# resero-labs/latok

Hardware: AMD Instinct MI355X
Metric: input UTF-8 GB/s tokenized (fused feature+split-mask path) (higher is better)
Workload: dtype u64

## Files before the change

latok_amd/csrc/api.cpp:

```cpp
#include <hip/hip_runtime.h>
#include <errno.h>
#include <fcntl.h>
#include <stdarg.h>
#include <stdio.h>
#include <stdlib.h>
#include <string.h>
#include <sys/mman.h>
#include <sys/stat.h>
#include <unistd.h>

#include <algorithm>
#include <array>
#include <atomic>
#include <chrono>
#include <mutex>
#include <new>
#include <string>
#include <thread>
#include <vector>

#include "../../include/latok_hip.h"
#include "corpus_gen.h"
#include "flow_hazards.h"
#include "kernels.h"
// ... 3266 lines not shown
    HIP_TRY(latok::launch_utf8_bytes(cps, n, (unsigned long long*)g.ws.scalar.p, g.stream));
    unsigned long long t = 0;
    HIP_TRY(hipMemcpyAsync(&t, g.ws.scalar.p, 8, hipMemcpyDeviceToHost, g.stream));
    HIP_TRY(hipStreamSynchronize(g.stream));
    *bytes_out = (int64_t)t;
    return LATOK_OK;
}

int latok_debug_set_scan_epoch(unsigned epoch) {
    LATOK_ENTER();
    g.ws.scan_epoch = epoch & 0x3FFFFu;
    return LATOK_OK;
}

extern "C" int latok_debug_limits(int64_t* out, int n) {
    const int64_t v[19] = {latok::kTile, latok::kWPB, latok::kNarrowWPB, latok::kSegMax, latok::kOneSegTiles, latok::kFastTailTiles,
                           kSmallChars, kSmallStrings, latok::kCompressWaves, latok::kFeatWaves, latok::kFeatRound, latok::kFeatRoundTm,
                           latok::kFeatFormThresh, latok::kFeatWinBytes, latok::kHashWaveBytes, latok::scan_small_max(),
                           latok::utf8_block_bytes(), latok::kCountProbeMax, latok::kCountAccEntries};
    if (!out || n < 0) return fail(LATOK_ERR_INVALID, "NULL output");
    const int k = n < 19 ? n : 19;
    for (int i = 0; i < k; ++i) out[i] = v[i];
    return k;
}

extern "C" int latok_debug_terms_limits(int64_t* out, int n) {
    const int64_t v[2] = {latok::kTermsTile, latok::kTermsRowMax};
    if (!out || n < 0) return fail(LATOK_ERR_INVALID, "NULL output");
    const int k = n < 2 ? n : 2;
    for (int i = 0; i < k; ++i) out[i] = v[i];
    return k;
}

extern "C" int latok_debug_wordpiece_limits(int64_t* out, int n) {
    const int64_t v[4] = {latok::kWpBlock, latok::scan_chunk(), kWpMaxPrefix, kWpMaxChars};
    if (!out || n < 0) return fail(LATOK_ERR_INVALID, "NULL output");
    const int k = n < 4 ? n : 4;
    for (int i = 0; i < k; ++i) out[i] = v[i];
    return k;
}

static int put_plan(const latok::LaunchPlan& L, int64_t n_tiles, int64_t* out, int n) {
    const int64_t v[12] = {L.n_cu_eff, L.seg_tiles, L.n_segs, L.rounds, L.grid, L.one_launch ? 0 : L.grid, L.fast_tail, L.pf, L.wpb, L.nw,
                           L.one_launch, n_tiles};
    const int k = n < 12 ? n : 12;
    for (int i = 0; i < k; ++i) out[i] = v[i];
    return k;
}

extern "C" int latok_debug_plan(int64_t n_tiles, int n_cu, int in_flow, int mode, int64_t* out, int n) {
    if (!out || n < 0 || n_tiles < 1 || n_cu < 1 || mode < latok::kModeBits || mode > latok::kModeValuesRules)
        return fail(LATOK_ERR_INVALID, "n_tiles >= 1, n_cu >= 1, mode 0..%d", latok::kModeValuesRules);
    latok::LaunchPlan L;
    latok::plan_launch(n_tiles, n_cu, in_flow != 0, mode, one_segment_enabled(), &L);
    return put_plan(L, n_tiles, out, n);
}

extern "C" int latok_debug_set_plan_cus(int n_cu) {
    LATOK_ENTER();
    int rc = need_init(g);
    if (rc) return rc;
    if (n_cu != 0 && (n_cu < 8 || n_cu > g.n_cu)) return fail(LATOK_ERR_INVALID, "plan CUs must be 0 or 8..%d", g.n_cu);
    g.plan_cus = n_cu;
    return LATOK_OK;
}

// ... 1010 lines not shown
```

latok_amd/csrc/kernels.h:

```cpp
#ifndef LATOK_KERNELS_H
#define LATOK_KERNELS_H
#include <hip/hip_runtime.h>
#include <stdint.h>

#include "split_code.h"

namespace latok {

constexpr int kTile = 4096;
constexpr int kTblShift = 7;
constexpr int kStage1Len = 8705;
constexpr int kStage1Pad = 8720;
constexpr int kStage2Len = 255 * 128;
constexpr int kTablesLdsBytes = kStage1Pad + kStage2Len;
constexpr int kB6Stage1Len = LK_B6_STAGE1_LEN;
constexpr int kB6Stage1Bytes = (kB6Stage1Len * 2 + 1023) / 1024 * 1024;
constexpr int kB6MaxBlocks = 400;
constexpr int kB6Stage2Bytes = kB6MaxBlocks * 64;
constexpr int kB6TablesBytes = kB6Stage1Bytes + kB6Stage2Bytes;
static_assert(kB6Stage1Bytes % 1024 == 0 && kB6Stage2Bytes % 1024 == 0 && kB6Stage1Bytes <= kTablesLdsBytes, "byte space keeps its stage 1 where the other modes keep both stages");
constexpr int kStageBytes = 64 * 80;
constexpr int kWaveLdsBytes = kStageBytes + 16 + 65 * 8 + 8;

constexpr int kModeBits = 0;
// ... 90 lines not shown
__device__ __forceinline__ int64_t device_total(const int64_t* p, int64_t bound) {
    const int64_t t = *p;
    return t < 0 ? 0 : (t > bound ? bound : t);
}
#endif

struct FeatParams {
    const uint8_t* codes;
    const int64_t* row_off;
    int64_t n_str, total, n_tiles;
    const uint64_t* bits;
    const uint64_t* kept;
    const int64_t* tile_rank;
    const int64_t* tile_cnt;
    const uint16_t* word_pref;
    const int64_t* tile_first;
    const uint64_t* space;
    int8_t* features;
    void* spans4;
    bool out32;
    const int64_t* n_tokens_dev;
    int64_t cap;
    DoneSignal done;
    DeviceTotal dt;
};
hipError_t launch_features_tiles(const FeatParams& P, int n_cu, hipStream_t st);

void plan_segments(int64_t n_tiles, int n_cu, int* seg_tiles, int64_t* n_segs);
constexpr int64_t kOneSegTiles = 24;
constexpr int64_t kFastTailTiles = 256;
constexpr int kNarrowWPB = 16;
constexpr int kCpsPrefetchRows = 2;
constexpr int kCpsPrefetchRowsFlow = 6;
struct LaunchPlan {
    int n_cu_eff;
    int seg_tiles;
    int64_t n_segs;
    int64_t rounds;
    int grid;
    int fast_tail;
    int pf;
    int wpb;
    int nw;
    int one_launch;
};
void plan_launch(int64_t n_tiles, int n_cu, bool in_flow, int mode, bool one_launch_ok, LaunchPlan* L);
hipError_t launch_tile_index(const SplitParams& P, hipStream_t st);
hipError_t launch_split_tiles(const SplitParams& P, int mode, const LaunchPlan& L, hipStream_t st);
hipError_t launch_resolve_fix(const SplitParams& P, int mode, const LaunchPlan& L, hipStream_t st);
hipError_t launch_one_segment(const SplitParams& P, int mode, hipStream_t st);
hipError_t launch_small_batch(const SplitParams& P, bool rules, int kind, bool out32, void* counts, void* items, int8_t* features,
                              int64_t* n_items, unsigned long long* done, unsigned long long seq, hipStream_t st);
hipError_t launch_any_nonzero(const int8_t* a1, const int8_t* a2, int64_t n, int* flags, hipStream_t st);

hipError_t launch_parse_matrix(const uint32_t* cps, int64_t n, const uint8_t* t1, const uint8_t* t2cls,
                               const uint16_t* cw, int8_t* out, hipStream_t st);
constexpr int kSmallMatrixChars = 4096;
hipError_t launch_parse_matrix_small(const uint32_t* cps, int n, const uint8_t* t1, const uint8_t* t2cls, const uint16_t* cw,
                                     int8_t* out, unsigned long long* done, unsigned long long seq, hipStream_t st);
hipError_t launch_combine_rows(const uint8_t* m, int64_t stride_r, int64_t stride_c, int64_t cols, const int8_t* idx,
                               int idx_ndim, int irows, int icols, int8_t* out, hipStream_t st,
                               unsigned long long* done = nullptr, unsigned long long seq = 0);
hipError_t launch_small_block_mask(const SplitParams& P, unsigned long long* done, unsigned long long seq, hipStream_t st);
hipError_t launch_rebase_rows(int64_t* row, int64_t n, int64_t base, hipStream_t st);
int64_t scan_blocks(int64_t n);
hipError_t launch_exclusive_scan(const int64_t* in, int64_t n, int64_t* out, int64_t* total, int64_t* block_tot,
                                 hipStream_t st, int64_t* total_host = nullptr);
int64_t count_blocks(int64_t n_words);
int64_t scan_chunk();
hipError_t launch_word_counts_scan(bool spans, const uint64_t* bits, const uint64_t* space, int64_t n_words, int64_t total,
                                   uint64_t* kept, int64_t* tile_cnt, uint16_t* word_pref, int64_t* tile_rank,
                                   unsigned long long* chain, unsigned* ticket, unsigned epoch, int64_t* total_dev,
                                   int64_t* total_host, int* err, hipStream_t st, DeviceTotal dt = DeviceTotal{nullptr, nullptr});
hipError_t launch_string_counts(bool out32, const uint64_t* mask, const int64_t* tile_rank, const uint16_t* word_pref,
// ... 108 lines not shown
```

latok_amd/csrc/split_kernels.hip:

```cpp
#include <hip/hip_runtime.h>
#include <stdint.h>
#include <stdlib.h>

#include "bitscan.h"
#include "feat_records.h"
#include "kernels.h"
#include "tile_core.h"

namespace latok {

#ifdef LATOK_STAMPS
__device__ unsigned long long g_stamp_sum[16];
__device__ unsigned long long g_stamp_cnt;
#endif

__device__ __forceinline__ Fn64 fn_then(Fn64 f1, Fn64 f2) {
    Fn64 f;
    const bool c1 = f1.a <= kNegInf64, c2 = f2.a <= kNegInf64;
    if (c2) { f.a = kNegInf64; f.b = f2.b; return f; }
    f.a = c1 ? kNegInf64 : f1.a + f2.a;
    const long long c = f1.b + f2.a;
    f.b = c > f2.b ? c : f2.b;
    return f;
}
// ... 203 lines not shown
            for (int j = 0; j < kLazyPer; ++j) {
                const int row = g * kLazyPer + j;
                if (row < kLazyRows)
                    __builtin_amdgcn_global_load_lds((gptr_t)(P.t1 + 1024 * row + 16 * lane), (lptr_t)(L.tables + 1024 * row), 16, 0, 0);
            }
            __builtin_amdgcn_s_waitcnt(0x0F70);
        }
        __hip_atomic_fetch_add(&L.ctl[1], 1, __ATOMIC_RELEASE, __HIP_MEMORY_SCOPE_WORKGROUP);
    }
    while (__hip_atomic_load(&L.ctl[1], __ATOMIC_ACQUIRE, __HIP_MEMORY_SCOPE_WORKGROUP) < 64 * kLazyGrabs) __builtin_amdgcn_s_sleep(2);
}

template <int MODE = kModeBits>
__device__ __forceinline__ TileLds wave_lds(uint8_t* lds, int wave) {
    TileLds L;
    L.t1 = lds;
    L.t2 = lds + kStage1Pad;
    uint8_t* const w = lds + lds_shift(MODE);
    uint8_t* mine = wave < kWPB ? w + kLdsWaves + wave * kWaveLdsBytes : lds + lds_total(MODE) + (wave - kWPB) * kWaveLdsBytes;
    L.stage = mine;
    L.halo = mine + kStageBytes;
    L.bw = reinterpret_cast<lk_u64*>(mine + kStageBytes + 16);
    L.lut = lds;
    L.ltab = lds + kLdsLeadTab;
    L.tables = lds;
    L.ctl = reinterpret_cast<int*>(w + kLdsMisc) + 16;
    L.t1b = lds;
    L.t2b = lds + kB6Stage1Bytes;
    L.ctab = mode_base(MODE) == kModeBytes ? lds + kLdsByteCodes : L.lut + kSliceLutBytes;
    L.small_bits = L.small_space = nullptr;
    return L;
}

template <int MODE, bool FAST_TAIL = false, int WPB = kWPB, int PF = kCpsPrefetchRows>
__device__ __forceinline__ void run_segment(const SplitParams& P, uint8_t* lds, int64_t seg, int tid, int lane,
                                            int wave, bool tables LATOK_STAMP_PARAM) {
    const int S = P.seg_tiles;
    const TileLds L = wave_lds<MODE>(lds, wave);
    int4* sm = reinterpret_cast<int4*>(lds + lds_shift(MODE) + kLdsSumm);
    ScanLdsT<WPB>& scan = *reinterpret_cast<ScanLdsT<WPB>*>(lds + lds_shift(MODE) + kLdsScan);

    const int64_t T0 = seg * S;
    const int64_t T1 = min(T0 + S, P.n_tiles);
    const int n_seg = (int)(T1 - T0);
    int64_t tfv = 0;
    if (wave + WPB * lane < n_seg) tfv = P.tile_first[T0 + wave + WPB * lane];
    tfv = tfv < 0 ? 0 : (tfv > P.n_str ? P.n_str : tfv);
    if (tables) __syncthreads();
    constexpr bool kDefer = mode_writes_bits(MODE) && !mode_is_bytes(MODE);
    lk_u64 obuf[8];
    int slot = 0, k_first = wave;
    const int64_t n_words = (P.total + 63) >> 6;
    auto flush = [&]() {
#pragma unroll
        for (int j = 0; j < 8; ++j) {
            if (j < slot) {
                const int64_t w = (T0 + k_first + j * WPB) * 64 + lane;
                if (w < n_words) P.bits_out[w] = obuf[j];
            }
        }
        slot = 0;
    };
    auto put = [&](lk_u64 w, int k) {
        if (slot == 0) k_first = k;
#pragma unroll
        for (int j = 0; j < 8; ++j) obuf[j] = (j == slot) ? w : obuf[j];
        if (++slot == 8) flush();
    };
    CpsPrefetch pf;
    pf.valid = false;
    for (int k = wave, j = 0; k < n_seg; k += WPB, ++j) {
        const lk_u64 w = process_tile<MODE, kDefer, false, FAST_TAIL, PF>(P, L, T0 + k, lane_read64(tfv, j), 0, -1, true, &sm[k], lane LATOK_STAMP_ARG
                                                                      , MODE == kModeBits && !FAST_TAIL ? &pf : nullptr, k + WPB < n_seg ? T0 + k + WPB : (int64_t)-1
                                                                      );
        if (kDefer) put(w, k);
#ifdef LATOK_STAMPS
        stamp_acc[0] += 1;
#endif
    }
    if (kDefer) flush();
    __syncthreads();
    {
        Fn64 f = fn_identity();
        Hd64 h = hd_identity();
        if (tid < n_seg) {
            const int4 s = sm[tid];
            P.summ[T0 + tid] = s;
            f = fn_of(s);
            h.h = s.z; h.c = s.w & 1;
        }
        Fn64 ef, tfn; Hd64 eh, th;
        block_scan<WPB>(f, h, scan, &ef, &eh, &tfn, &th);
        if (tid == 0) { P.seg_fn[seg] = tfn; P.seg_hd[seg] = th; }
    }
    __syncthreads();
}

template <int MODE, bool FAST_TAIL = false, int PF = kCpsPrefetchRows>
__global__ __launch_bounds__(tile_wpb(MODE) * 64) void k_tiles_main(SplitParams P) {
    constexpr int WPB = tile_wpb(MODE);
    __shared__ __attribute__((aligned(16))) uint8_t lds[lds_total_tiles(MODE)];
    const int tid = threadIdx.x;
    const int lane = tid & 63;
    const int wave = __builtin_amdgcn_readfirstlane(tid >> 6);
    if (blockIdx.x == 0 && tid == 0) *P.fix_count = 0;

    bool tables = MODE != kModeBlockMask;
    if (tables) {
        if (mode_base(MODE) == kModeBytes) load_tables_ascii_bytes(lds, P);
        else load_tables<WPB * 64, MODE>(lds, P);
    }
#ifdef LATOK_STAMPS
    unsigned long long stamp_acc[16];
    for (int i = 0; i < 16; ++i) stamp_acc[i] = 0;
#endif
    for (int64_t seg = blockIdx.x; seg < P.n_segs; seg += gridDim.x) {
        run_segment<MODE, FAST_TAIL, WPB, PF>(P, lds, seg, tid, lane, wave, tables LATOK_STAMP_ARG);
        tables = false;
    }
#ifdef LATOK_STAMPS
    if (lane == 0)
        for (int i = 0; i < 16; ++i) atomicAdd(&g_stamp_sum[i], stamp_acc[i]);
#endif
}

template <int MODE, int NW, bool ONE>
__device__ __forceinline__ void resolve_segments(const SplitParams& P, uint8_t* lds, int tid, int lane, int wave) {
    const int S = P.seg_tiles;
    ScanLdsT<NW>& scan = *reinterpret_cast<ScanLdsT<NW>*>(lds + lds_shift(MODE) + kLdsScan);
    int* misc = reinterpret_cast<int*>(lds + lds_shift(MODE) + kLdsMisc);
    int* fix_t = reinterpret_cast<int*>(lds + lds_shift(MODE) + kLdsTf);
    int2* fix_in = reinterpret_cast<int2*>(lds + lds_shift(MODE) + kLdsSumm);
    bool tables_loaded = ONE;

    for (int64_t seg = ONE ? 0 : (int64_t)blockIdx.x; seg < (ONE ? 1 : P.n_segs); seg += ONE ? 1 : (int64_t)gridDim.x) {
        const int64_t T0 = seg * S;
        const int64_t T1 = min(T0 + S, P.n_tiles);
        const int n_seg = (int)(T1 - T0);
        if (tid == 0) misc[0] = 0;
        const int64_t t = T0 + tid;
        int4 s = make_int4(0, 0, 0, 0);
        if (tid < n_seg) s = P.summ[t];
        Fn64 pf = fn_identity();
        Hd64 sh = hd_identity();
        if (P.n_segs > 1) {
            const int64_t per = (P.n_segs + NW * 64 - 1) / (NW * 64);
            const int64_t lo = min((int64_t)tid * per, P.n_segs), hi = min(lo + per, P.n_segs);
            Fn64 f = fn_identity();
            Hd64 h = hd_identity();
            for (int64_t j = lo; j < hi; ++j) {
// ... 411 lines not shown
    if (s > kSegMax) s = kSegMax;
    *seg_tiles = (int)s;
    *n_segs = (n_tiles + s - 1) / s;
}

void plan_launch(int64_t n_tiles, int n_cu, bool in_flow, int mode, bool one_launch_ok, LaunchPlan* L) {
    const int wpb = tile_wpb(mode);
    int n_cu_eff = n_cu;
    if (in_flow && n_cu >= 64) {
        const int cand[3] = {n_cu * 7 / 8, n_cu * 13 / 16, n_cu * 3 / 4};
        int best = cand[0], best_fill = -1;
        for (int c = 0; c < 3; ++c) {
            int st_ = 0;
            int64_t ns_ = 0;
            plan_segments(n_tiles, cand[c], &st_, &ns_);
            const int fill = (st_ - 1) % wpb + 1;
            if (fill * 2 >= wpb) { best = cand[c]; break; }
            if (fill > best_fill) { best = cand[c]; best_fill = fill; }
        }
        n_cu_eff = best;
    }
    if (n_cu_eff < 8) n_cu_eff = n_cu < 8 ? n_cu : 8;
    L->n_cu_eff = n_cu_eff;
    plan_segments(n_tiles, n_cu_eff, &L->seg_tiles, &L->n_segs);
    L->one_launch = one_launch_ok && n_tiles <= kOneSegTiles && (mode == kModeBits || mode == kModeRules);
    if (L->one_launch) {
        L->seg_tiles = (int)(n_tiles < kOneSegTiles ? kOneSegTiles : n_tiles);
        L->n_segs = 1;
    }
    L->grid = L->one_launch ? 1 : (int)(L->n_segs < n_cu ? (L->n_segs < 1 ? 1 : L->n_segs) : n_cu);
    L->rounds = (L->n_segs + L->grid - 1) / L->grid;
    L->fast_tail = !L->one_launch && n_tiles <= kFastTailTiles && (mode == kModeBits || mode == kModeRules);
    L->pf = mode == kModeBits && in_flow && !L->fast_tail && !L->one_launch ? kCpsPrefetchRowsFlow : kCpsPrefetchRows;
    L->wpb = L->one_launch ? kWPB : wpb;
    const bool narrow_resolve = mode == kModeBits || mode == kModeBytes || mode == kModeLatin1 || mode == kModeUcs2;
    L->nw = L->one_launch || !narrow_resolve ? kWPB : (L->seg_tiles <= 128 ? 2 : (L->seg_tiles <= 256 ? 4 : kWPB));
}

hipError_t launch_split_tiles(const SplitParams& P, int mode, const LaunchPlan& L, hipStream_t st) {
    const dim3 grid(L.grid), block(kWPB * 64);
    if (mode == kModeBits && L.pf == kCpsPrefetchRowsFlow) hipLaunchKernelGGL((k_tiles_main<kModeBits, false, kCpsPrefetchRowsFlow>), grid, block, 0, st, P);
    else if (mode == kModeBits && L.fast_tail) hipLaunchKernelGGL((k_tiles_main<kModeBits, true>), grid, block, 0, st, P);
    else if (mode == kModeRules && L.fast_tail) hipLaunchKernelGGL((k_tiles_main<kModeRules, true>), grid, block, 0, st, P);
    else if (mode == kModeBits) hipLaunchKernelGGL((k_tiles_main<kModeBits>), grid, block, 0, st, P);
    else if (mode == kModeValues) hipLaunchKernelGGL((k_tiles_main<kModeValues>), grid, block, 0, st, P);
    else if (mode == kModeRules) hipLaunchKernelGGL((k_tiles_main<kModeRules>), grid, block, 0, st, P);
    else if (mode == kModeBytes) hipLaunchKernelGGL((k_tiles_main<kModeBytes>), grid, dim3(tile_wpb(kModeBytes) * 64), 0, st, P);
    else if (mode == kModeLatin1) hipLaunchKernelGGL((k_tiles_main<kModeLatin1>), grid, dim3(tile_wpb(kModeLatin1) * 64), 0, st, P);
    else if (mode == kModeUcs2) hipLaunchKernelGGL((k_tiles_main<kModeUcs2>), grid, dim3(tile_wpb(kModeUcs2) * 64), 0, st, P);
    else if (mode == kModeBytesRules) hipLaunchKernelGGL((k_tiles_main<kModeBytesRules>), grid, block, 0, st, P);
    else if (mode == kModeLatin1Rules) hipLaunchKernelGGL((k_tiles_main<kModeLatin1Rules>), grid, block, 0, st, P);
    else if (mode == kModeUcs2Rules) hipLaunchKernelGGL((k_tiles_main<kModeUcs2Rules>), grid, block, 0, st, P);
    else if (mode == kModeValuesRules) hipLaunchKernelGGL((k_tiles_main<kModeValuesRules>), grid, block, 0, st, P);
    else hipLaunchKernelGGL((k_tiles_main<kModeBlockMask>), grid, block, 0, st, P);
    return hipGetLastError();
}

hipError_t launch_one_segment(const SplitParams& P, int mode, hipStream_t st) {
    if (P.n_segs != 1 || P.seg_tiles < P.n_tiles || P.n_tiles > kOneSegTiles || (mode != kModeBits && mode != kModeRules))
        return hipErrorInvalidValue;
    if (mode == kModeBits) hipLaunchKernelGGL((k_one_segment<kModeBits>), dim3(1), dim3(kWPB * 64), 0, st, P);
    else hipLaunchKernelGGL((k_one_segment<kModeRules>), dim3(1), dim3(kWPB * 64), 0, st, P);
    return hipGetLastError();
}

hipError_t launch_resolve_fix(const SplitParams& P, int mode, const LaunchPlan& L, hipStream_t st) {
    if (L.nw * 64 < P.seg_tiles) return hipErrorInvalidValue;
    const dim3 grid(L.grid), block(kWPB * 64);
#define LATOK_RESOLVE_NW(M)                                                                            \
    if (L.nw == 2) hipLaunchKernelGGL((k_resolve_fix<M, 2>), grid, dim3(128), 0, st, P);               \
    else if (L.nw == 4) hipLaunchKernelGGL((k_resolve_fix<M, 4>), grid, dim3(256), 0, st, P);          \
    else hipLaunchKernelGGL((k_resolve_fix<M, kWPB>), grid, block, 0, st, P)
    if (mode == kModeBits) { LATOK_RESOLVE_NW(kModeBits); }
    else if (mode == kModeValues) hipLaunchKernelGGL((k_resolve_fix<kModeValues, kWPB>), grid, block, 0, st, P);
    else if (mode == kModeRules) hipLaunchKernelGGL((k_resolve_fix<kModeRules, kWPB>), grid, block, 0, st, P);
    else if (mode == kModeBytesRules) hipLaunchKernelGGL((k_resolve_fix<kModeBytesRules, kWPB>), grid, block, 0, st, P);
    else if (mode == kModeLatin1Rules) hipLaunchKernelGGL((k_resolve_fix<kModeLatin1Rules, kWPB>), grid, block, 0, st, P);
// ... 23 lines not shown
```

latok_amd/csrc/tile_core.h:

```cpp
#ifndef LATOK_TILE_CORE_H
#define LATOK_TILE_CORE_H
#include <hip/hip_runtime.h>
#include <stdint.h>

#include "kernels.h"
#include "lane_math.h"
#include "utf8_decode.h"
#include "wave_ops.h"

namespace latok {

#ifdef LATOK_STAMPS
#define LATOK_STAMP(k)                                                                           \
    do {                                                                                         \
        __builtin_amdgcn_sched_barrier(0);                                                       \
        unsigned long long t_;                                                                   \
        asm volatile("s_memtime %0\n\ts_waitcnt lgkmcnt(0)" : "=s"(t_)::"memory");            \
        __builtin_amdgcn_sched_barrier(0);                                                       \
        if ((k) > 0) stamp_acc[(k)] += t_ - stamp_prev;                                          \
        stamp_prev = t_;                                                                         \
    } while (0)
#define LATOK_STAMP_ARG , stamp_acc
#define LATOK_STAMP_PARAM , unsigned long long* stamp_acc
#define LATOK_STAMP_NULL , nullptr
// ... 226 lines not shown
    return *reinterpret_cast<const uint2*>(ltab + ((W & 0xFFu) << 3));
}
__device__ __forceinline__ bool lead_index(uint2 q, uint32_t W, uint32_t* off2, uint32_t* R) {
    lk_lead_entry e;
    e.sel = q.x; e.hi0 = q.y;
    uint32_t o;
    const bool bad = lk_lead_index(e, W, &o, R);
    *off2 = min(o, 2u * (uint32_t)(kB6Stage1Len - 1));
    return bad;
}

template <int Q>
__device__ __forceinline__ uint32_t bytes_slot_window(const uint32_t (&w)[5], uint32_t m, uint32_t* r8_out) {
    const uint32_t r8 = (uint32_t)__builtin_ctz(m | 0x80000000u) & 24u;
    *r8_out = r8;
    return __builtin_amdgcn_alignbit(w[Q + 1], w[Q], r8);
}

__device__ __forceinline__ uint32_t bytes_halo_load(const uint8_t* __restrict__ u8, int64_t t0, int64_t total, int lane) {
    uint32_t hb = 0;
    if (lane == 0) {
        if (t0 > 0) hb = *reinterpret_cast<const uint32_t*>(u8 + t0 - 4);
    } else if (lane < 12) {
        const int64_t q = t0 + kTile + (lane - 1);
        if (q < total) hb = u8[q];
    }
    return hb;
}

constexpr int kCpsPrefetchMax = kCpsPrefetchRowsFlow;
struct CpsPrefetch {
    u32x4 v[kCpsPrefetchMax];
    bool valid;
};

__device__ __forceinline__ bool bytes_phase1(const SplitParams& P, const TileLds& L, int64_t t0, int lane
#ifdef LATOK_STAMPS
                                             , unsigned long long* stamp_acc, unsigned long long& stamp_prev
#endif
                                             ) {
    const int64_t total = P.total;
    const uint8_t* __restrict__ u8 = P.u8;
    uint32_t hb = bytes_halo_load(u8, t0, total, lane);
    u32x4 v[4];
    if (t0 + kTile <= total) {
        const u32x4* src = reinterpret_cast<const u32x4*>(u8 + t0) + lane;
#pragma unroll
        for (int i = 0; i < 4; ++i) v[i] = __builtin_nontemporal_load(src + 64 * i);
    } else {
#pragma unroll 1
        for (int i = 0; i < 4; ++i) {
            uint32_t d[4] = {0, 0, 0, 0};
            const int64_t p = t0 + 1024 * i + 16 * lane;
            for (int j = 0; j < 16; ++j)
                if (p + j < total) d[j >> 2] |= (uint32_t)u8[p + j] << (8 * (j & 3));
            v[i].x = d[0]; v[i].y = d[1]; v[i].z = d[2]; v[i].w = d[3];
        }
    }
    uint32_t hi_bits = (hb | v[0].x | v[0].y | v[0].z | v[0].w) & 0x80808080u;
    if (__all(hi_bits == 0u)) {
#pragma unroll
        for (int i = 1; i < 4; ++i) hi_bits |= (v[i].x | v[i].y | v[i].z | v[i].w) & 0x80808080u;
    }
    if (lane < 2) *reinterpret_cast<lk_u64*>(L.halo + 8u * lane) = 0ull;
    const bool all_ascii = __all(hi_bits == 0u);
    wave_lds_sync();
    LATOK_STAMP(11);
// ... 139 lines not shown
                }
            }
            *reinterpret_cast<uint4*>(L.stage + stage_addr(1024u * (i0 + a) + 16u * lane)) = make_uint4(out[a][0], out[a][1], out[a][2], out[a][3]);
        }
    }
    LATOK_STAMP(13);
    {
        const int k = lane - 1;
        const bool in_win = lane >= 1 && lane < 9 && t0 + kTile + k < total;
        const uint32_t b1 = (uint32_t)dpp_mov<kDppWaveShl1, 0xF>(0, (int)hb) & 0xFFu;
        const uint32_t b2 = (uint32_t)dpp_mov<kDppWaveShl1, 0xF>(0, (int)b1) & 0xFFu;
        const uint32_t b3 = (uint32_t)dpp_mov<kDppWaveShl1, 0xF>(0, (int)b2) & 0xFFu;
        const uint32_t W = (hb & 0xFFu) | (b1 << 8) | (b2 << 16) | (b3 << 24);
        const uint32_t b0 = W & 0xFFu;
        const uint32_t my_code = classify1_b6(L.t1b, L.t2b, b0 < 0x80u ? b0 : utf8_cp_of(W));
        if (in_win) L.halo[8 + k] = (uint8_t)(u8_is_cont(b0) ? LK_CODE_CONT : my_code);
    }
    return false;
}

__device__ __forceinline__ void bytes_word_context(const TileLds& L, int lane, lk_halo_bytes* hb, bool* next_has_cont, uint32_t* own_code,
                                                   int* own_left) {
    hb->next_codes = lane < 63 ? *reinterpret_cast<const lk_u64*>(L.stage + 80u * lane + 80u) : *reinterpret_cast<const lk_u64*>(L.halo + 8);
    hb->next_B = (uint32_t)(L.bw[lane + 1] & 0xFFFFull);
    const lk_u64 y = hb->next_codes ^ 0x8080808080808080ull;
    *next_has_cont = (~(((y & 0x7F7F7F7F7F7F7F7Full) + 0x7F7F7F7F7F7F7F7Full) | y) & 0x8080808080808080ull) != 0ull;
    lk_owner_before(lane > 0 ? *reinterpret_cast<const uint32_t*>(L.stage + 80u * lane - 20u) : 0u, own_code, own_left);
    if (lane == 0) {
        *own_code = L.halo[0];
        *own_left = L.halo[4];
    }
    hb->prev = *own_code;
}
template <int MODE, bool DEFER = false, bool SMALL = false>
__device__ __forceinline__ lk_u64 tile_phase2(const SplitParams& P, const TileLds& L, int64_t t, int q_in, int tail_zero,
                                            bool write_summary, int4* summ_l, int lane, bool raw_stage, bool ascii_tile
#ifdef LATOK_STAMPS
                                            , unsigned long long* stamp_acc, unsigned long long& stamp_prev
#endif
                                            ) {
    const int64_t t0 = t * kTile;
    const int64_t total = P.total;
    const lk_u64 B = L.bw[lane];
    const int64_t base = t0 + 64 * (int64_t)lane;
    lk_local loc;
    lk_rule_counts counts;
    lk_u64 space_plane = 0;
    lk_u64 cont_plane = 0;
    int no_patch = 0;
    if (MODE == kModeBlockMask) {
        lk_u64 st = 0, sp = 0;
#pragma unroll
        for (int k = 0; k < 16; ++k) {
            const int64_t p = base + 4 * k;
            uint32_t w1 = 0, w2 = 0;
            if (p + 4 <= total) {
                w1 = *reinterpret_cast<const uint32_t*>(P.bm_a1 + p);
                w2 = *reinterpret_cast<const uint32_t*>(P.bm_a2 + p);
            } else {
                for (int b = 0; b < 4; ++b)
                    if (p + b < total) {
                        w1 |= (uint32_t)(uint8_t)P.bm_a1[p + b] << (8 * b);
                        w2 |= (uint32_t)(uint8_t)P.bm_a2[p + b] << (8 * b);
                    }
            }
            const uint32_t n1 = ((((w1 & 0x7F7F7F7Fu) + 0x7F7F7F7Fu) | w1) & 0x80808080u) >> 7;
            const uint32_t n2 = ((((w2 & 0x7F7F7F7Fu) + 0x7F7F7F7Fu) | w2) & 0x80808080u) >> 7;
            st |= (lk_u64)(((n1 * 0x00204081u) >> 21) & 0xFu) << (4 * k);
            sp |= (lk_u64)(((n2 * 0x00204081u) >> 21) & 0xFu) << (4 * k);
// ... 56 lines not shown
            uint32_t own_code;
            int own_left;
            bytes_word_context(L, lane, &hb, &next_has_cont, &own_code, &own_left);
            no_patch = __ballot(C != 0ull || next_has_cont) != 0ull;
            if (!no_patch) {
                lk_halo ha;
                ha.prev = h.prev;
                ha.next0 = (uint32_t)(hb.next_codes & 0xFFull);
                ha.next1 = (uint32_t)((hb.next_codes >> 8) & 0xFFull);
                if (mode_rules(MODE)) loc = lk_rules_generic(plane, ha, B, Bn, P.rules);
                else loc = lk_rules(lk_decode(plane), ha, B, Bn);
                space_plane = loc.S;
            } else if (mode_rules(MODE)) {
                lk_smear_planes<0x37u>(plane, C, own_code, own_left);
                hb.prev = own_code;
                loc = lk_rules_generic_bytes(plane, C, hb, B, P.rules, &space_plane);
            } else if (__ballot(lk_rules_bytes_weird(plane, C, hb.next_codes)) == 0ull) {
                lk_smear_planes<0x37u>(plane, C, own_code, own_left);
                hb.prev = own_code;
                loc = lk_rules_bytes_fast(plane, C, hb, B, &space_plane);
            } else {
                lk_smear_planes<0x37u>(plane, C, own_code, own_left);
                hb.prev = own_code;
                loc = lk_rules_bytes_general(plane, C, hb, B, &space_plane);
            }
        } else if (mode_rules(MODE)) {
            loc = lk_rules_generic(plane, h, B, Bn, P.rules, MODE == kModeValuesRules ? &counts : nullptr);
        } else {
            const lk_feat f = lk_decode(plane);
            loc = lk_rules(f, h, B, Bn);
        }
    }
    LATOK_STAMP(4);
    lk_fwd fw = lk_forward(loc.start, loc.S, B);

    const lk_qfn inc = qfn_wave_scan(lk_qfn_of(fw));
    lk_qfn exc;
    exc.a = dpp_mov<kDppWaveShr1, 0xF>(0, inc.a);
    exc.b = dpp_mov<kDppWaveShr1, 0xF>(0, inc.b);
    const int r = lk_qfn_apply(exc, q_in);
    lk_qfn tile_fn;
    tile_fn.a = lane_read(inc.a, 63);
    tile_fn.b = lane_read(inc.b, 63);
    if (r > 0) lk_apply_extra(fw, r);
    LATOK_STAMP(5);

    if (write_summary) {
        const lk_u64 cl = loc.S | B;
        const lk_u64 closing_lanes = __ballot(cl != 0);
        const int first_lane = closing_lanes ? lk_ctz(closing_lanes) : 64;
        const int contrib = lane < first_lane ? lk_popc(loc.start) : (lane == first_lane ? fw.head_starts : 0);
        const int head = __ballot(contrib != 0) ? wave_sum(contrib) : 0;
        int c_rel = kTile, p_rel = 0, tail_keep = 0;
        if (closing_lanes) {
            const int last_lane = 63 - __builtin_clzll(closing_lanes);
            const int my_first = cl ? 64 * lane + lk_ctz(cl) : 0;
            const int top = cl ? 63 - __builtin_clzll(cl) : 0;
            const int s_top = (int)((loc.S >> top) & 1ull);
            c_rel = lane_read(my_first, first_lane);
            p_rel = lane_read(64 * lane + top + s_top, last_lane);
            tail_keep = lane_read(1 - s_top, last_lane);
        }
        int head_sym, tail_sym;
        if (mode_base(MODE) == kModeBytes && no_patch) {
            const int64_t lo_w = 64 * (int64_t)lane;
            const lk_u64 in_head = c_rel >= lo_w + 64 ? ~0ull : (c_rel <= lo_w ? 0ull : ((1ull << (c_rel - lo_w)) - 1ull));
            const lk_u64 in_tail = p_rel <= lo_w ? ~0ull : (p_rel >= lo_w + 64 ? 0ull : (~0ull << (p_rel - lo_w)));
            head_sym = __ballot((loc.sym & in_head) != 0ull) != 0ull;
            tail_sym = __ballot((loc.sym & in_tail) != 0ull) != 0ull;
        } else {
            const int hs_pos = c_rel > 0 ? c_rel - 1 : 0;
            head_sym = c_rel > 0 ? lane_read((int)((loc.sym >> (hs_pos & 63)) & 1ull), hs_pos >> 6) : 0;
            tail_sym = lane_read((int)(loc.sym >> 63), 63);
        }
        if (lane == 0) {
            const int geom = (closing_lanes != 0) | (c_rel << 1) | (p_rel << 14) | (head_sym << 27) | (tail_keep << 28) |
                             (tail_sym << 29) | (no_patch << 30);
            *summ_l = make_int4(tile_fn.a, tile_fn.b, head, geom);
        }
    }

    LATOK_STAMP(6);
    const lk_u64 zall = fw.zs | fw.zb;
    const int z0_next = dpp_mov<kDppWaveShl1, 0xF>(0, (int)(zall & 1ull));
    const lk_bwd bw = lk_backward_prepare(zall, loc.S, B, z0_next);
    const int tz = tail_zero >= 0 ? tail_zero : (lk_qfn_apply(tile_fn, q_in) > 0);
    const lk_u64 G = lk_rev(__ballot(bw.g)), Pm = lk_rev(__ballot(bw.p));
    const lk_u64 X = G | Pm, Y = G;
    const lk_u64 carries_in = (X + Y + (lk_u64)tz) ^ X ^ Y;
    const int cin = (int)((carries_in >> (63 - lane)) & 1ull);
    const lk_u64 cleared = lk_backward_fill(bw, cin, loc.S);

    LATOK_STAMP(7);
    lk_u64 out_word = 0;
    if (base < total) {
        const int64_t remain = total - base;
        const lk_u64 valid = remain >= 64 ? ~0ull : ((1ull << remain) - 1ull);
        const lk_u64 keep = ~cleared;
        if (mode_writes_bits(MODE)) {
            out_word = ((loc.raw & keep) | loc.sym | B) & valid;
            uint64_t* const bits_out = SMALL ? L.small_bits : P.bits_out;
            uint64_t* const space_out = SMALL ? L.small_space : P.space_out;
            if (!DEFER) bits_out[base >> 6] = out_word;
            if (space_out) space_out[base >> 6] = (mode_is_bytes(MODE) ? space_plane : loc.S) & valid;
        } else {
            uint8_t* dst = P.values_out + base;
            const int n = remain >= 64 ? 64 : (int)remain;
#pragma unroll 1
            for (int w = 0; w < 16; ++w) {
                uint32_t packed = 0;
                if (MODE == kModeBlockMask) {
                    packed = ((uint32_t)((keep >> (4 * w)) & 0xFull) * 0x00204081u) & 0x01010101u;
                    if (base == 0 && w == 0) {
                        const int first = (P.bm_flags[0] != 0 && P.bm_flags[1] == 0) ? 0 : 1;
                        packed = (packed & ~0xFFu) | (uint32_t)first;
                    }
                } else {
#pragma unroll
                    for (int b = 0; b < 4; ++b) {
                        const int i = 4 * w + b;
                        int v, vy;
                        if (MODE == kModeValuesRules) {
                            v = vy = 0;
#pragma unroll
                            for (int c = 0; c < LK_COUNT_BITS; ++c) {
                                v |= (int)((counts.split[c] >> i) & 1) << c;
// ... 12 lines not shown
                }
                if (4 * w + 4 <= n) {
                    *reinterpret_cast<uint32_t*>(dst + 4 * w) = packed;
                } else {
                    for (int b = 0; b < 4 && 4 * w + b < n; ++b) dst[4 * w + b] = (uint8_t)(packed >> (8 * b));
                }
            }
        }
    }
    if (mode_base(MODE) == kModeBytes && !SMALL && P.lead_out) {
        const int64_t remain = total - base;
        const lk_u64 valid = remain >= 64 ? ~0ull : (remain <= 0 ? 0ull : ((1ull << remain) - 1ull));
        const lk_u64 leadw = ~cont_plane & valid;
        const int cnt = lk_popc(leadw);
        int inc = cnt;
        inc += dpp_mov<kDppRowShr1, 0xF>(0, inc);
        inc += dpp_mov<kDppRowShr2, 0xF>(0, inc);
        inc += dpp_mov<kDppRowShr4, 0xF>(0, inc);
        inc += dpp_mov<kDppRowShr8, 0xF>(0, inc);
        inc += dpp_mov<kDppRowBcast15, 0xA>(0, inc);
        inc += dpp_mov<kDppRowBcast31, 0xC>(0, inc);
        if (base < total) {
            P.lead_out[base >> 6] = leadw;
            P.lead_pref_out[base >> 6] = (uint16_t)(inc - cnt);
        }
        if (lane == 63) P.lead_cnt_out[t] = inc;
    }
    LATOK_STAMP(8);
    wave_lds_sync();
    return out_word;
}


template <int MODE, bool DEFER = false, bool SMALL = false, bool FAST_TAIL = false, int PF = kCpsPrefetchRows>
__device__ __forceinline__ lk_u64 process_tile(const SplitParams& P, const TileLds& L, int64_t t, int64_t idx0, int q_in,
                                             int tail_zero, bool write_summary, int4* summ_l, int lane
#ifdef LATOK_STAMPS
                                             , unsigned long long* stamp_acc = nullptr
#endif
                                             , CpsPrefetch* pf = nullptr, int64_t t_next = -1
                                             ) {
#ifdef LATOK_STAMPS
    unsigned long long stamp_prev = 0, stamp_dummy[16];
    if (!stamp_acc) stamp_acc = stamp_dummy;
#endif
    const int64_t t0 = t * kTile;
    const int64_t total = P.total;
    const uint32_t st_lane = 4u * lane + 16u * ((uint32_t)lane >> 4);
    bool raw_stage = mode_base(MODE) == kModeLatin1;
    bool ascii_tile = false;
    bool tile_not_ascii = false;
    LATOK_STAMP(0);

    int64_t ro = idx0 + lane <= P.n_str ? P.row_off[idx0 + lane] : INT64_MAX;
    uint32_t halo_cp = 0xFFFFFFFFu;
    if (MODE != kModeBlockMask && !mode_is_bytes(MODE) && lane < 3) {
        const int64_t hp = lane == 0 ? t0 - 1 : t0 + kTile + (lane - 1);
        if (hp >= 0 && hp < total) halo_cp = P.cps[hp];
    }

    if (MODE == kModeBlockMask) {
    } else if (mode_base(MODE) == kModeLatin1) {
        ascii_tile = units_phase1<1>(P, L, t0, lane);
    } else if (mode_base(MODE) == kModeUcs2) {
        units_phase1<2>(P, L, t0, lane);
    } else if (mode_base(MODE) == kModeBytes) {
        raw_stage = bytes_phase1(P, L, t0, lane
// ... 11 lines not shown
        if (full) {
#pragma unroll
            for (int i = 0; i < 16; ++i) v[i] = __builtin_nontemporal_load(src + 64 * i);
        } else {
            const int64_t last_blk = (total - 1) & ~(int64_t)3;
            n_rows = (int)((total - t0 + 255) >> 8);
#pragma unroll
            for (int i = 0; i < 16; ++i) {
                if (i < n_rows) {
                    int64_t p = t0 + 256 * i + 4 * (int64_t)lane;
                    p = p < last_blk ? p : last_blk;
                    v[i] = __builtin_nontemporal_load(reinterpret_cast<const u32x4*>(P.cps + p));
                }
            }
        }
        uint32_t* codes = P.codes_out ? reinterpret_cast<uint32_t*>(P.codes_out + t0) + lane : nullptr;
#pragma unroll
        for (int i = 0; i < 16; ++i) {
            uint32_t c = 0;
            if (i < n_rows) {
                c = classify4(L.t1, L.t2, v[i]);
                if (!full) {
                    const int64_t remain = remain0 - 256 * i;
                    c &= remain >= 4 ? 0xFFFFFFFFu : (remain <= 0 ? 0u : ((1u << (8 * (int)remain)) - 1u));
                }
            }
            *reinterpret_cast<uint32_t*>(L.stage + st_lane + 320u * i) = c;
            if (codes) codes[64 * i] = c;
        }
    } else if (t0 + kTile <= total) {
        u32x4 v[16];
        const u32x4* src = reinterpret_cast<const u32x4*>(P.cps + t0) + lane;
        constexpr int R = PF;
        const bool pre = R > 0 && pf && pf->valid;
#pragma unroll
        for (int i = 0; i < 16; ++i) {
            if (i < R && pre) v[i] = pf->v[i < R ? i : 0];
            else v[i] = __builtin_nontemporal_load(src + 64 * i);
        }
        LATOK_STAMP(1);
        uint32_t* codes = P.codes_out ? reinterpret_cast<uint32_t*>(P.codes_out + t0) + lane : nullptr;
#pragma unroll
        for (int i = 0; i < 16; ++i) {
            const uint32_t c = classify4(L.t1, L.t2, v[i], &tile_not_ascii);
            *reinterpret_cast<uint32_t*>(L.stage + st_lane + 320u * i) = c;
            if (codes) codes[64 * i] = c;
        }
    } else {
        uint32_t* codes = P.codes_out ? reinterpret_cast<uint32_t*>(P.codes_out + t0) + lane : nullptr;
#pragma unroll 1
        for (int i = 0; i < 16; ++i) {
            const int64_t p = t0 + 256 * i + 4 * lane;
            u32x4 v;
            v.x = p + 0 < total ? P.cps[p + 0] : 0xFFFFFFFFu;
            v.y = p + 1 < total ? P.cps[p + 1] : 0xFFFFFFFFu;
            v.z = p + 2 < total ? P.cps[p + 2] : 0xFFFFFFFFu;
            v.w = p + 3 < total ? P.cps[p + 3] : 0xFFFFFFFFu;
            const uint32_t c = classify4(L.t1, L.t2, v);
            *reinterpret_cast<uint32_t*>(L.stage + st_lane + 320u * i) = c;
            if (codes) codes[64 * i] = c;
        }
    }
    if (MODE != kModeBlockMask && !mode_is_bytes(MODE) && lane < 3) L.halo[lane] = (uint8_t)classify1(L.t1, L.t2, halo_cp);
    L.bw[lane] = 0;
    if (lane == 0) L.bw[64] = 0;
    LATOK_STAMP(2);
    wave_lds_sync();
    for (;;) {
        const int64_t rel = ro - t0;
        if (rel >= 0 && rel < kTile + 64) atomicOr(&L.bw[rel >> 6], 1ull << (rel & 63));
        const int64_t last = lane_read64(ro, 63);
        if (last >= t0 + kTile + 64) break;
        idx0 += 64;
        ro = idx0 + lane <= P.n_str ? P.row_off[idx0 + lane] : INT64_MAX;
    }
    wave_lds_sync();
    LATOK_STAMP(3);
    if (MODE == kModeBits && pf) {
        __builtin_amdgcn_s_waitcnt(0x0F70);
        pf->valid = false;
        const bool want = true;
        if (want && t_next >= 0 && (t_next + 1) * kTile <= total) {
            const u32x4* nsrc = reinterpret_cast<const u32x4*>(P.cps + t_next * kTile) + lane;
#pragma unroll
            for (int i = 0; i < PF; ++i) pf->v[i] = __builtin_nontemporal_load(nsrc + 64 * i);
            pf->valid = true;
        }
    }

    return tile_phase2<MODE, DEFER, SMALL>(P, L, t, q_in, tail_zero, write_summary, summ_l, lane, raw_stage, ascii_tile
#ifdef LATOK_STAMPS
                                    , stamp_acc, stamp_prev
#endif
                                    );
}

}
#endif
```

Before: 1510.

## Interleave next-tile codepoint loads and classification into phase-2 seams

Adds a drain mask that, at up to four seams inside tile_phase2, classifies the already-prefetched rows of the next tile into LDS staging and issues loads for the following rows. This spreads the next tile's global loads across the current tile's scan phases, so memory latency overlaps compute instead of being paid mostly at tile start. The next tile then skips the rows already classified and carries over its non-ASCII flag. It adds waitcnt stalls and LDS writes in the middle of phase 2, raises register pressure, and risks staging-buffer hazards if the wave's stage area is still in use when it is overwritten.

```diff
diff --git a/latok_amd/csrc/api.cpp b/latok_amd/csrc/api.cpp
--- a/latok_amd/csrc/api.cpp
+++ b/latok_amd/csrc/api.cpp
@@ -3322,6 +3322,15 @@
     return k;
 }
 
+extern "C" int latok_debug_readahead(int64_t* out, int n) {
+    LATOK_ENTER();
+    if (!out || n < 0) return fail(LATOK_ERR_INVALID, "NULL output");
+    const int64_t v[4] = {g.inited && g.last.valid ? g.last.plan.drains : -1, latok::kCpsDrainMask, latok::kCpsDrainMaskFlow, 4};
+    const int k = n < 4 ? n : 4;
+    for (int i = 0; i < k; ++i) out[i] = v[i];
+    return k;
+}
+
 extern "C" int latok_debug_wordpiece_limits(int64_t* out, int n) {
     const int64_t v[4] = {latok::kWpBlock, latok::scan_chunk(), kWpMaxPrefix, kWpMaxChars};
     if (!out || n < 0) return fail(LATOK_ERR_INVALID, "NULL output");
diff --git a/latok_amd/csrc/kernels.h b/latok_amd/csrc/kernels.h
--- a/latok_amd/csrc/kernels.h
+++ b/latok_amd/csrc/kernels.h
@@ -146,6 +146,14 @@
 constexpr int kNarrowWPB = 16;
 constexpr int kCpsPrefetchRows = 2;
 constexpr int kCpsPrefetchRowsFlow = 6;
+#ifndef LATOK_DRAIN_MASK
+#define LATOK_DRAIN_MASK 0xF
+#endif
+#ifndef LATOK_DRAIN_MASK_FLOW
+#define LATOK_DRAIN_MASK_FLOW 0x0
+#endif
+constexpr int kCpsDrainMask = LATOK_DRAIN_MASK;
+constexpr int kCpsDrainMaskFlow = LATOK_DRAIN_MASK_FLOW;
 struct LaunchPlan {
     int n_cu_eff;
     int seg_tiles;
@@ -154,6 +162,7 @@
     int grid;
     int fast_tail;
     int pf;
+    int drains;
     int wpb;
     int nw;
     int one_launch;
diff --git a/latok_amd/csrc/split_kernels.hip b/latok_amd/csrc/split_kernels.hip
--- a/latok_amd/csrc/split_kernels.hip
+++ b/latok_amd/csrc/split_kernels.hip
@@ -259,7 +259,7 @@
     return L;
 }
 
-template <int MODE, bool FAST_TAIL = false, int WPB = kWPB, int PF = kCpsPrefetchRows>
+template <int MODE, bool FAST_TAIL = false, int WPB = kWPB, int PF = kCpsPrefetchRows, int DM = 0>
 __device__ __forceinline__ void run_segment(const SplitParams& P, uint8_t* lds, int64_t seg, int tid, int lane,
                                             int wave, bool tables LATOK_STAMP_PARAM) {
     const int S = P.seg_tiles;
@@ -295,9 +295,9 @@
         if (++slot == 8) flush();
     };
     CpsPrefetch pf;
-    pf.valid = false;
+    pf.valid = pf.not_ascii = false;
     for (int k = wave, j = 0; k < n_seg; k += WPB, ++j) {
-        const lk_u64 w = process_tile<MODE, kDefer, false, FAST_TAIL, PF>(P, L, T0 + k, lane_read64(tfv, j), 0, -1, true, &sm[k], lane LATOK_STAMP_ARG
+        const lk_u64 w = process_tile<MODE, kDefer, false, FAST_TAIL, PF, DM>(P, L, T0 + k, lane_read64(tfv, j), 0, -1, true, &sm[k], lane LATOK_STAMP_ARG
                                                                       , MODE == kModeBits && !FAST_TAIL ? &pf : nullptr, k + WPB < n_seg ? T0 + k + WPB : (int64_t)-1
                                                                       );
         if (kDefer) put(w, k);
@@ -323,7 +323,7 @@
     __syncthreads();
 }
 
-template <int MODE, bool FAST_TAIL = false, int PF = kCpsPrefetchRows>
+template <int MODE, bool FAST_TAIL = false, int PF = kCpsPrefetchRows, int DM = 0>
 __global__ __launch_bounds__(tile_wpb(MODE) * 64) void k_tiles_main(SplitParams P) {
     constexpr int WPB = tile_wpb(MODE);
     __shared__ __attribute__((aligned(16))) uint8_t lds[lds_total_tiles(MODE)];
@@ -342,7 +342,7 @@
     for (int i = 0; i < 16; ++i) stamp_acc[i] = 0;
 #endif
     for (int64_t seg = blockIdx.x; seg < P.n_segs; seg += gridDim.x) {
-        run_segment<MODE, FAST_TAIL, WPB, PF>(P, lds, seg, tid, lane, wave, tables LATOK_STAMP_ARG);
+        run_segment<MODE, FAST_TAIL, WPB, PF, DM>(P, lds, seg, tid, lane, wave, tables LATOK_STAMP_ARG);
         tables = false;
     }
 #ifdef LATOK_STAMPS
@@ -820,6 +820,7 @@
     L->rounds = (L->n_segs + L->grid - 1) / L->grid;
     L->fast_tail = !L->one_launch && n_tiles <= kFastTailTiles && (mode == kModeBits || mode == kModeRules);
     L->pf = mode == kModeBits && in_flow && !L->fast_tail && !L->one_launch ? kCpsPrefetchRowsFlow : kCpsPrefetchRows;
+    L->drains = mode != kModeBits || L->fast_tail || L->one_launch ? 0 : (L->pf == kCpsPrefetchRowsFlow ? kCpsDrainMaskFlow : kCpsDrainMask);
     L->wpb = L->one_launch ? kWPB : wpb;
     const bool narrow_resolve = mode == kModeBits || mode == kModeBytes || mode == kModeLatin1 || mode == kModeUcs2;
     L->nw = L->one_launch || !narrow_resolve ? kWPB : (L->seg_tiles <= 128 ? 2 : (L->seg_tiles <= 256 ? 4 : kWPB));
@@ -827,10 +828,10 @@
 
 hipError_t launch_split_tiles(const SplitParams& P, int mode, const LaunchPlan& L, hipStream_t st) {
     const dim3 grid(L.grid), block(kWPB * 64);
-    if (mode == kModeBits && L.pf == kCpsPrefetchRowsFlow) hipLaunchKernelGGL((k_tiles_main<kModeBits, false, kCpsPrefetchRowsFlow>), grid, block, 0, st, P);
+    if (mode == kModeBits && L.pf == kCpsPrefetchRowsFlow) hipLaunchKernelGGL((k_tiles_main<kModeBits, false, kCpsPrefetchRowsFlow, kCpsDrainMaskFlow>), grid, block, 0, st, P);
     else if (mode == kModeBits && L.fast_tail) hipLaunchKernelGGL((k_tiles_main<kModeBits, true>), grid, block, 0, st, P);
     else if (mode == kModeRules && L.fast_tail) hipLaunchKernelGGL((k_tiles_main<kModeRules, true>), grid, block, 0, st, P);
-    else if (mode == kModeBits) hipLaunchKernelGGL((k_tiles_main<kModeBits>), grid, block, 0, st, P);
+    else if (mode == kModeBits) hipLaunchKernelGGL((k_tiles_main<kModeBits, false, kCpsPrefetchRows, kCpsDrainMask>), grid, block, 0, st, P);
     else if (mode == kModeValues) hipLaunchKernelGGL((k_tiles_main<kModeValues>), grid, block, 0, st, P);
     else if (mode == kModeRules) hipLaunchKernelGGL((k_tiles_main<kModeRules>), grid, block, 0, st, P);
     else if (mode == kModeBytes) hipLaunchKernelGGL((k_tiles_main<kModeBytes>), grid, dim3(tile_wpb(kModeBytes) * 64), 0, st, P);
diff --git a/latok_amd/csrc/tile_core.h b/latok_amd/csrc/tile_core.h
--- a/latok_amd/csrc/tile_core.h
+++ b/latok_amd/csrc/tile_core.h
@@ -282,7 +282,30 @@
 struct CpsPrefetch {
     u32x4 v[kCpsPrefetchMax];
     bool valid;
+    bool not_ascii;
 };
+constexpr int kCpsDrainSeams = 4;
+constexpr int cps_drains_before(int dm, int s) { return __builtin_popcount((unsigned)dm & ((1u << s) - 1u)); }
+constexpr int cps_rows_done(int r, int dm) { return cps_drains_before(dm, kCpsDrainSeams) * r < 16 ? cps_drains_before(dm, kCpsDrainSeams) * r : 16; }
+
+template <int R, int J>
+__device__ __forceinline__ void cps_drain(const SplitParams& P, const TileLds& L, CpsPrefetch* pf, int64_t t_next, int lane) {
+    constexpr int lo = J * R < 16 ? J * R : 16, hi = lo + R < 16 ? lo + R : 16, nhi = hi + R < 16 ? hi + R : 16;
+    if (lo >= hi || !pf->valid) return;
+    if (J == 0) wave_lds_sync();
+    __builtin_amdgcn_s_waitcnt(0x0F70);
+    const uint32_t st_lane = 4u * lane + 16u * ((uint32_t)lane >> 4);
+    uint32_t* codes = P.codes_out ? reinterpret_cast<uint32_t*>(P.codes_out + t_next * kTile) + lane : nullptr;
+#pragma unroll
+    for (int i = lo; i < hi; ++i) {
+        const uint32_t c = classify4(L.t1, L.t2, pf->v[i - lo], &pf->not_ascii);
+        *reinterpret_cast<uint32_t*>(L.stage + st_lane + 320u * i) = c;
+        if (codes) codes[64 * i] = c;
+    }
+    const u32x4* nsrc = reinterpret_cast<const u32x4*>(P.cps + t_next * kTile) + lane;
+#pragma unroll
+    for (int i = hi; i < nhi; ++i) pf->v[i - hi] = __builtin_nontemporal_load(nsrc + 64 * i);
+}
 
 __device__ __forceinline__ bool bytes_phase1(const SplitParams& P, const TileLds& L, int64_t t0, int lane
 #ifdef LATOK_STAMPS
@@ -488,9 +511,10 @@
     }
     hb->prev = *own_code;
 }
-template <int MODE, bool DEFER = false, bool SMALL = false>
+template <int MODE, bool DEFER = false, bool SMALL = false, int R = 0, int DM = 0>
 __device__ __forceinline__ lk_u64 tile_phase2(const SplitParams& P, const TileLds& L, int64_t t, int q_in, int tail_zero,
-                                            bool write_summary, int4* summ_l, int lane, bool raw_stage, bool ascii_tile
+                                            bool write_summary, int4* summ_l, int lane, bool raw_stage, bool ascii_tile,
+                                            CpsPrefetch* pf, int64_t t_next
 #ifdef LATOK_STAMPS
                                             , unsigned long long* stamp_acc, unsigned long long& stamp_prev
 #endif
@@ -613,6 +637,7 @@
         }
     }
     LATOK_STAMP(4);
+    if constexpr ((DM & 1) != 0) cps_drain<R, cps_drains_before(DM, 0)>(P, L, pf, t_next, lane);
     lk_fwd fw = lk_forward(loc.start, loc.S, B);
 
     const lk_qfn inc = qfn_wave_scan(lk_qfn_of(fw));
@@ -625,6 +650,7 @@
     tile_fn.b = lane_read(inc.b, 63);
     if (r > 0) lk_apply_extra(fw, r);
     LATOK_STAMP(5);
+    if constexpr ((DM & 2) != 0) cps_drain<R, cps_drains_before(DM, 1)>(P, L, pf, t_next, lane);
 
     if (write_summary) {
         const lk_u64 cl = loc.S | B;
@@ -662,6 +688,7 @@
     }
 
     LATOK_STAMP(6);
+    if constexpr ((DM & 4) != 0) cps_drain<R, cps_drains_before(DM, 2)>(P, L, pf, t_next, lane);
     const lk_u64 zall = fw.zs | fw.zb;
     const int z0_next = dpp_mov<kDppWaveShl1, 0xF>(0, (int)(zall & 1ull));
     const lk_bwd bw = lk_backward_prepare(zall, loc.S, B, z0_next);
@@ -673,6 +700,7 @@
     const lk_u64 cleared = lk_backward_fill(bw, cin, loc.S);
 
     LATOK_STAMP(7);
+    if constexpr ((DM & 8) != 0) cps_drain<R, cps_drains_before(DM, 3)>(P, L, pf, t_next, lane);
     lk_u64 out_word = 0;
     if (base < total) {
         const int64_t remain = total - base;
@@ -751,7 +779,7 @@
 }
 
 
-template <int MODE, bool DEFER = false, bool SMALL = false, bool FAST_TAIL = false, int PF = kCpsPrefetchRows>
+template <int MODE, bool DEFER = false, bool SMALL = false, bool FAST_TAIL = false, int PF = kCpsPrefetchRows, int DM = 0>
 __device__ __forceinline__ lk_u64 process_tile(const SplitParams& P, const TileLds& L, int64_t t, int64_t idx0, int q_in,
                                              int tail_zero, bool write_summary, int4* summ_l, int lane
 #ifdef LATOK_STAMPS
@@ -829,16 +857,20 @@
         u32x4 v[16];
         const u32x4* src = reinterpret_cast<const u32x4*>(P.cps + t0) + lane;
         constexpr int R = PF;
+        constexpr int kDone = (MODE == kModeBits && !FAST_TAIL) ? cps_rows_done(R, DM) : 0;
         const bool pre = R > 0 && pf && pf->valid;
 #pragma unroll
         for (int i = 0; i < 16; ++i) {
-            if (i < R && pre) v[i] = pf->v[i < R ? i : 0];
+            if (i < kDone && pre) continue;
+            if (i < kDone + R && pre) v[i] = pf->v[i >= kDone && i < kDone + R ? i - kDone : 0];
             else v[i] = __builtin_nontemporal_load(src + 64 * i);
         }
         LATOK_STAMP(1);
+        if (kDone > 0 && pre) tile_not_ascii = pf->not_ascii;
         uint32_t* codes = P.codes_out ? reinterpret_cast<uint32_t*>(P.codes_out + t0) + lane : nullptr;
 #pragma unroll
         for (int i = 0; i < 16; ++i) {
+            if (i < kDone && pre) continue;
             const uint32_t c = classify4(L.t1, L.t2, v[i], &tile_not_ascii);
             *reinterpret_cast<uint32_t*>(L.stage + st_lane + 320u * i) = c;
             if (codes) codes[64 * i] = c;
@@ -882,10 +914,11 @@
 #pragma unroll
             for (int i = 0; i < PF; ++i) pf->v[i] = __builtin_nontemporal_load(nsrc + 64 * i);
             pf->valid = true;
-        }
-    }
-
-    return tile_phase2<MODE, DEFER, SMALL>(P, L, t, q_in, tail_zero, write_summary, summ_l, lane, raw_stage, ascii_tile
+            pf->not_ascii = false;
+        }
+    }
+
+    return tile_phase2<MODE, DEFER, SMALL, PF, (MODE == kModeBits && !FAST_TAIL) ? DM : 0>(P, L, t, q_in, tail_zero, write_summary, summ_l, lane, raw_stage, ascii_tile, pf, t_next
 #ifdef LATOK_STAMPS
                                     , stamp_acc, stamp_prev
 #endif
```

Result: no change. 1509 (-0.1%).
